# Azure/gpu-provisioner

Measured on AMD Instinct MI355X. Metric: nodeclaims_per_min, higher is better.
Workload: dtype n/a; 1 GPU; model=MI355X NodeClaim provisioning (karpenter CloudProvider contract), vm_sku=Standard_ND128isr_MI355X_v6, concurrent_nodeclaims=8, cloud=in-memory fake AKS, zero latency (BASELINE config #1), apiserver=in-memory, server-side CRD validation on, cycle=create→Launched→Registered→Initialized(amd.com/gpu)→delete→gone, parallelism=single

## Files before the change

### __graft_entry__.py

```python
from __future__ import annotations

import os
import subprocess
import sys
import sysconfig

ROOT = os.path.dirname(os.path.abspath(__file__))
sys.path.insert(0, ROOT)

NATIVE_DIR = os.path.join(ROOT, "gpu_provisioner_amd", "_native")
LIB_PATH = os.path.join(NATIVE_DIR, "libmi355x_nodeagent.so")
HIP_SRC = os.path.join(ROOT, "nodeagent", "agent.hip")
EXTENSIONS = {
    "_jsontree": os.path.join(ROOT, "native", "jsontree.cpp"),
    "_objmodel": os.path.join(ROOT, "native", "objmodel.cpp"),
}


def build() -> None:
    os.makedirs(NATIVE_DIR, exist_ok=True)
    cmd = [
        "hipcc",
        "--offload-arch=gfx950",
        "-O3",
        "-shared",
        "-fPIC",
        HIP_SRC,
        "-o",
        LIB_PATH,
    ]
    print("+", " ".join(cmd), flush=True)
    subprocess.run(cmd, check=True)
    assert os.path.exists(LIB_PATH), f"{LIB_PATH} missing after build"

    for module, src in EXTENSIONS.items():
        ext_path = os.path.join(NATIVE_DIR, module + sysconfig.get_config_var("EXT_SUFFIX"))
        cmd = [
            os.environ.get("CXX", "c++"),
            "-O2",
            "-std=c++17",
            "-shared",
            "-fPIC",
            "-I" + sysconfig.get_paths()["include"],
            src,
            "-o",
            ext_path,
        ]
        print("+", " ".join(cmd), flush=True)
        subprocess.run(cmd, check=True)
        assert os.path.exists(ext_path), f"{ext_path} missing after build"

    import gpu_provisioner_amd
    from gpu_provisioner_amd._native import _jsontree, _objmodel
    from gpu_provisioner_amd.kube import objects

    if os.environ.get("GPU_PROVISIONER_PURE_PYTHON") != "1":
        assert objects.NATIVE_JSONTREE, "native JSON-tree extension built but not in use"
        assert objects.NATIVE_OBJMODEL, "native object-model extension built but not in use"
    from gpu_provisioner_amd.fake.harness import Harness
    from gpu_provisioner_amd.nodeagent import NodeAgent

    print(f"build OK: {LIB_PATH} ({os.path.getsize(LIB_PATH)} bytes)", flush=True)


def smoke() -> None:
    import asyncio

    from gpu_provisioner_amd.apis import v1 as karpv1
    from gpu_provisioner_amd.fake.harness import Harness

    async def provision_cycle() -> None:
        h = Harness(node_wait_interval=0.005).add_all_controllers(
            lifecycle_workers=32, termination_requeue=0.01,
            drain_requeue=0.01, instance_poll=0.01, gc_interval=30.0,
        )
        await h.start()
        try:
            await h.kube.create(h.make_nodeclaim("smoke1"))
            done = await h.wait_initialized("smoke1", timeout=30.0)
            assert karpv1.is_initialized(done), "nodeclaim not initialized"
            assert done["status"]["allocatable"][karpv1.AMD_GPU_RESOURCE] == "8"
            await h.kube.delete(karpv1.API_VERSION, karpv1.KIND_NODECLAIM, "smoke1")
            await h.wait_gone(karpv1.API_VERSION, karpv1.KIND_NODECLAIM, "smoke1", timeout=30.0)
        finally:
            await h.stop()

    asyncio.run(provision_cycle())
    print("smoke: provision+teardown cycle OK", flush=True)

    gpu_available = False
    try:
        import torch

        gpu_available = torch.cuda.is_available()
    except Exception:
        pass
    if gpu_available:
        from gpu_provisioner_amd.nodeagent import NodeAgent

        agent = NodeAgent()
        report = agent.check(bw_bytes=1 << 28)
        assert report.gpu_count >= 1, "no GPUs found by node agent"
        g0 = report.gpus[0]
        assert g0.healthy, f"node agent found problems: {g0.problems}"
        print(
            f"smoke: nodeagent gpu0 {g0.arch} hbm={g0.hbm_gb}GB "
            f"bw={g0.hbm_bw_gbs}GB/s sdma={g0.sdma_bw_gbs}GB/s all-checks=OK",
            flush=True,
        )
    else:
        print("smoke: no GPU present; native nodeagent check skipped", flush=True)


if __name__ == "__main__":
    build()
    smoke()
```

### gpu_provisioner_amd/fake/apiserver.py

```python
from __future__ import annotations

import asyncio
from collections import deque
import itertools
from collections import defaultdict
from typing import Any, AsyncIterator, Callable, Optional

from ..kube import objects as ko
from ..kube.client import (
    ADDED,
    DELETED,
    MODIFIED,
    AlreadyExistsError,
    APIError,
    ConflictError,
    GoneError,
    InvalidError,
    KubeClient,
    LabelSelector,
    NotFoundError,
    json_merge_patch,
    match_field_selector,
    merge_patch_owned,
)

_WATCH_HISTORY = 4096
_WATCH_BROKEN = "__WATCH_BROKEN__"

_SELECTABLE_FIELDS = {
    ("v1", "Pod"): {
        "spec.nodeName",
        "spec.schedulerName",
        "spec.restartPolicy",
        "spec.serviceAccountName",
        "spec.hostNetwork",
        "status.phase",
        "status.podIP",
        "status.nominatedNodeName",
    },
    ("v1", "Node"): {"spec.unschedulable"},
    ("v1", "Namespace"): {"status.phase", "name"},
    ("v1", "Secret"): {"type"},
    ("v1", "Event"): {
        "involvedObject.kind",
        "involvedObject.namespace",
        "involvedObject.name",
        "involvedObject.uid",
        "involvedObject.apiVersion",
        "involvedObject.resourceVersion",
        "involvedObject.fieldPath",
        "reason",
        "reportingComponent",
        "source",
        "type",
    },
}
_GENERIC_FIELDS = {"metadata.name", "metadata.namespace"}


def validate_field_selector(api_version: str, kind: str, selector: str) -> None:
    if not selector:
        return
    allowed = _GENERIC_FIELDS | _SELECTABLE_FIELDS.get((api_version, kind), set())
    for part in selector.split(","):
        part = part.strip()
        if not part:
            continue
        key = part.split("!=" if "!=" in part else "=", 1)[0].strip()
        if key not in allowed:
            raise InvalidError(f"field label not supported: {key}")


def _key(namespace: str, name: str) -> tuple:
    return (namespace or "", name)


def _gvk(api_version: str, kind: str) -> tuple:
    return (api_version, kind)


class InMemoryAPIServer:

    def __init__(self):
        self._store: dict = defaultdict(dict)
        self._rv = itertools.count(1)
        self._lock = asyncio.Lock()
        self._watchers: list = []
        self._history: deque = deque(maxlen=_WATCH_HISTORY)
        self.reactors: list = []
        self.validators: dict = {}
        self.eviction_reactor: Optional[Callable] = None
        self.evictions: list = []


    def _next_rv(self) -> str:
        return str(next(self._rv))

    def _fire_reactors(self, verb: str, gvk: tuple, payload: Any) -> None:
        for r in list(self.reactors):
            err = r(verb, gvk, payload)
            if err is not None:
                raise err

    def _broadcast(self, gvk: tuple, event_type: str, obj: dict) -> None:
        rv = int(obj["metadata"]["resourceVersion"])
        self._history.append((rv, gvk, event_type, obj))
        for wgvk, queue in self._watchers:
            if wgvk == gvk:
                queue.put_nowait((event_type, obj))

    def _bump(self, obj: dict) -> None:
        obj["metadata"]["resourceVersion"] = self._next_rv()

    def _validate(self, gvk: tuple, new: dict, old: Optional[dict]) -> None:
        fn = self.validators.get(gvk)
        if fn is None:
            return
        errs = fn(new, old)
        if errs:
            raise InvalidError(
                f"{gvk[1]} {ko.name_of(new)} is invalid: " + "; ".join(errs[:5])
            )


    async def get(self, api_version: str, kind: str, name: str, namespace: str) -> dict:
        async with self._lock:
            gvk = _gvk(api_version, kind)
            self._fire_reactors("get", gvk, name)
            obj = self._store[gvk].get(_key(namespace, name))
            if obj is None:
                raise NotFoundError(f"{kind} {namespace}/{name} not found")
            return ko.deep_copy(obj)

    async def list(
        self,
        api_version: str,
        kind: str,
        namespace: str,
        label_selector: str,
        field_selector: str,
    ) -> tuple:
        async with self._lock:
            gvk = _gvk(api_version, kind)
            validate_field_selector(api_version, kind, field_selector)
            self._fire_reactors("list", gvk, None)
            sel = LabelSelector.parse(label_selector) if label_selector else None
            out = []
            for (ns, _), obj in self._store[gvk].items():
                if namespace and ns != namespace:
                    continue
                if sel and not sel.matches(ko.labels_of(obj)):
                    continue
                if not match_field_selector(obj, field_selector):
                    continue
                out.append(ko.deep_copy(obj))
            return out, str(self._peek_rv())

    def _peek_rv(self) -> int:
        c = next(self._rv)
        self._rv = itertools.chain([c], self._rv)
        return c - 1

    async def create(self, obj: dict) -> dict:
        async with self._lock:
            api_version, kind = obj.get("apiVersion", ""), obj.get("kind", "")
            if not api_version or not kind or not ko.name_of(obj):
                raise InvalidError("apiVersion, kind and metadata.name are required")
            gvk = _gvk(api_version, kind)
            self._fire_reactors("create", gvk, obj)
            key = _key(ko.namespace_of(obj), ko.name_of(obj))
            if key in self._store[gvk]:
                raise AlreadyExistsError(f"{kind} {key[0]}/{key[1]} already exists")
            stored = ko.deep_copy(obj)
            m = ko.meta(stored)
            m["uid"] = m.get("uid") or ko.uuid4_str()
            m["creationTimestamp"] = m.get("creationTimestamp") or ko.now_rfc3339()
            m["generation"] = 1
            self._validate(gvk, stored, None)
            self._bump(stored)
            self._store[gvk][key] = stored
            if kind == "Event" and len(self._store[gvk]) > 20000:
                drop = next(iter(self._store[gvk]))
                del self._store[gvk][drop]
            self._broadcast(gvk, ADDED, stored)
            return ko.deep_copy(stored)

    async def update(self, obj: dict, subresource: str = "") -> dict:
        async with self._lock:
            api_version, kind = obj.get("apiVersion", ""), obj.get("kind", "")
            gvk = _gvk(api_version, kind)
            self._fire_reactors("update", gvk, obj)
            key = _key(ko.namespace_of(obj), ko.name_of(obj))
            cur = self._store[gvk].get(key)
            if cur is None:
                raise NotFoundError(f"{kind} {key[0]}/{key[1]} not found")
            rv = obj.get("metadata", {}).get("resourceVersion")
            if rv and rv != cur["metadata"]["resourceVersion"]:
                raise ConflictError(
                    f"{kind} {key[1]}: resourceVersion mismatch ({rv} != {cur['metadata']['resourceVersion']})"
                )
            return self._apply_update(gvk, key, cur, obj, subresource)

    def _apply_update(
        self, gvk: tuple, key: tuple, cur: dict, obj: dict, subresource: str, owned: bool = False
    ) -> dict:
        if subresource == "status":
            stored = {**cur, "metadata": {**cur["metadata"]}}
            stored["status"] = ko.deep_copy(obj.get("status", {}))
        else:
            if ko.is_deleting(cur):
                added = set(ko.finalizers_of(obj)) - set(ko.finalizers_of(cur))
                if added:
                    raise InvalidError(
                        "metadata.finalizers: Forbidden: no new finalizers can "
                        f"be added if the object is being deleted (added: {sorted(added)})"
                    )
            new = obj if owned else ko.deep_copy(obj)
            new["status"] = cur.get("status", {})
            nm = ko.meta(new)
            cm = cur["metadata"]
            for f in ("uid", "creationTimestamp", "generation", "deletionTimestamp"):
                if f in cm:
                    nm[f] = cm[f]
                else:
                    nm.pop(f, None)
            ns, cs = new.get("spec"), cur.get("spec")
            if ns is cs:
                pass
            elif ns != cs:
                nm["generation"] = cm.get("generation", 1) + 1
            elif "spec" in new:
                new["spec"] = cs
            stored = new
        self._validate(gvk, stored, cur)
        self._bump(stored)
        if ko.is_deleting(stored) and not ko.finalizers_of(stored) and subresource != "status":
            del self._store[gvk][key]
            self._broadcast(gvk, DELETED, stored)
        else:
            self._store[gvk][key] = stored
            self._broadcast(gvk, MODIFIED, stored)
        return ko.deep_copy(stored)

    async def patch(
        self,
        api_version: str,
        kind: str,
        name: str,
        patch: dict,
        namespace: str,
        subresource: str,
    ) -> dict:
        async with self._lock:
            gvk = _gvk(api_version, kind)
            self._fire_reactors("patch", gvk, name)
            key = _key(namespace, name)
            cur = self._store[gvk].get(key)
            if cur is None:
                raise NotFoundError(f"{kind} {namespace}/{name} not found")
            req_rv = (patch.get("metadata") or {}).get("resourceVersion")
            if req_rv and req_rv != cur["metadata"]["resourceVersion"]:
                raise ConflictError(
                    f"{kind} {name}: resourceVersion mismatch "
                    f"({req_rv} != {cur['metadata']['resourceVersion']})"
                )
            if subresource == "status":
                merged_status = json_merge_patch(cur.get("status", {}), patch.get("status", patch))
                return self._apply_update(gvk, key, cur, {"status": merged_status}, "status")
            merged = merge_patch_owned(cur, patch)
            merged.setdefault("metadata", {})["resourceVersion"] = cur["metadata"]["resourceVersion"]
            return self._apply_update(gvk, key, cur, merged, "", owned=True)

    async def delete(
        self,
        api_version: str,
        kind: str,
        name: str,
        namespace: str,
        uid_precondition: str = "",
        grace_period_seconds: Optional[int] = None,
    ) -> None:
        async with self._lock:
            gvk = _gvk(api_version, kind)
            self._fire_reactors("delete", gvk, name)
            key = _key(namespace, name)
            cur = self._store[gvk].get(key)
            if cur is None:
                raise NotFoundError(f"{kind} {namespace}/{name} not found")
            if uid_precondition and ko.uid_of(cur) != uid_precondition:
                raise ConflictError(f"{kind} {name}: uid precondition failed")
            if ko.finalizers_of(cur):
                if not ko.is_deleting(cur):
                    stored = {**cur, "metadata": {**cur["metadata"]}}
                    ko.meta(stored)["deletionTimestamp"] = ko.now_rfc3339()
                    self._bump(stored)
                    self._store[gvk][key] = stored
                    self._broadcast(gvk, MODIFIED, stored)
                return
            stored = {**cur, "metadata": {**cur["metadata"]}}
            ko.meta(stored)["deletionTimestamp"] = ko.now_rfc3339()
            self._bump(stored)
            del self._store[gvk][key]
            self._broadcast(gvk, DELETED, stored)

    async def evict(self, pod: dict, grace_period_seconds: Optional[int]) -> None:
        async with self._lock:
            if self.eviction_reactor is not None:
                err = self.eviction_reactor(pod)
                if err is not None:
                    raise err
            gvk = _gvk("v1", "Pod")
            key = _key(ko.namespace_of(pod), ko.name_of(pod))
            cur = self._store[gvk].get(key)
            if cur is None:
                raise NotFoundError(f"Pod {key[0]}/{key[1]} not found")
            self.evictions.append(key)
            stored = ko.deep_copy(cur)
            ko.meta(stored)["deletionTimestamp"] = ko.now_rfc3339()
            self._bump(stored)
            if ko.finalizers_of(cur):
                self._store[gvk][key] = stored
                self._broadcast(gvk, MODIFIED, stored)
            else:
                del self._store[gvk][key]
                self._broadcast(gvk, DELETED, stored)

    def subscribe(self, api_version: str, kind: str, resource_version: str) -> tuple:
        gvk = _gvk(api_version, kind)
        queue: asyncio.Queue = asyncio.Queue()
        if resource_version:
            rv = int(resource_version)
            if self._history:
                oldest = self._history[0][0]
                if rv + 1 < oldest and any(True for _ in self._store[gvk]):
                    raise GoneError(f"resourceVersion {rv} too old")
            for erv, egvk, etype, eobj in self._history:
                if egvk == gvk and erv > rv:
                    queue.put_nowait((etype, ko.deep_copy(eobj)))
        entry = (gvk, queue)
        self._watchers.append(entry)

        def unsubscribe():
            try:
                self._watchers.remove(entry)
            except ValueError:
                pass

        return queue, unsubscribe

    def break_watches(self) -> int:
        broken = 0
        for _, queue in list(self._watchers):
            queue.put_nowait((_WATCH_BROKEN, None))
            broken += 1
        return broken


class InMemoryClient(KubeClient):

    def __init__(self, server: InMemoryAPIServer):
        self.server = server

    async def get(self, api_version: str, kind: str, name: str, namespace: str = "") -> dict:
        return await self.server.get(api_version, kind, name, namespace)

    async def list(
        self,
# ... 78 lines not shown
```

### native/jsontree.cpp

```cpp
#define PY_SSIZE_T_CLEAN
#include <Python.h>

namespace {


inline bool is_container(PyObject* o) {
    return PyDict_CheckExact(o) || PyList_CheckExact(o);
}

PyObject* copy_tree(PyObject* o) {
    if (PyDict_CheckExact(o)) {
        if (Py_EnterRecursiveCall(" while copying a JSON tree")) return nullptr;
        PyObject* out = PyDict_Copy(o);
        if (out != nullptr) {
            Py_ssize_t pos = 0;
            PyObject *k, *v;
            while (PyDict_Next(out, &pos, &k, &v)) {
                if (!is_container(v)) continue;
                PyObject* nv = copy_tree(v);
                if (nv == nullptr || PyDict_SetItem(out, k, nv) < 0) {
                    Py_XDECREF(nv);
                    Py_CLEAR(out);
                    break;
                }
                Py_DECREF(nv);
            }
        }
        Py_LeaveRecursiveCall();
        return out;
    }
    if (PyList_CheckExact(o)) {
        if (Py_EnterRecursiveCall(" while copying a JSON tree")) return nullptr;
        PyObject* out = PyList_GetSlice(o, 0, PyList_GET_SIZE(o));
        if (out != nullptr) {
            Py_ssize_t n = PyList_GET_SIZE(out);
            for (Py_ssize_t i = 0; i < n; i++) {
                PyObject* v = PyList_GET_ITEM(out, i);
                if (!is_container(v)) continue;
                PyObject* nv = copy_tree(v);
                if (nv == nullptr) {
                    Py_CLEAR(out);
                    break;
                }
                PyList_SET_ITEM(out, i, nv);
                Py_DECREF(v);
            }
        }
        Py_LeaveRecursiveCall();
        return out;
    }
    Py_INCREF(o);
    return o;
}

PyObject* py_deep_copy(PyObject*, PyObject* obj) { return copy_tree(obj); }


PyObject* dict_of(PyObject* target) {
    if (target == nullptr || !PyDict_Check(target)) return PyDict_New();
    if (PyDict_CheckExact(target)) return PyDict_Copy(target);
    return PyObject_CallOneArg((PyObject*)&PyDict_Type, target);
}

PyObject* merge(PyObject* target, PyObject* patch, bool owned);

int merge_item(PyObject* out, PyObject* k, PyObject* v, bool owned) {
    if (v == Py_None) {
        if (PyDict_DelItem(out, k) < 0) {
            if (!PyErr_ExceptionMatches(PyExc_KeyError)) return -1;
            PyErr_Clear();
        }
        return 0;
    }
    PyObject* nv;
    if (PyDict_Check(v)) {
        PyObject* sub = PyDict_GetItemWithError(out, k);
        if (sub == nullptr && PyErr_Occurred()) return -1;
        Py_XINCREF(sub);
        nv = merge(sub, v, owned);
        Py_XDECREF(sub);
    } else if (owned) {
        nv = copy_tree(v);
    } else {
        Py_INCREF(v);
        nv = v;
    }
    if (nv == nullptr) return -1;
    int rc = PyDict_SetItem(out, k, nv);
    Py_DECREF(nv);
    return rc;
}

PyObject* merge(PyObject* target, PyObject* patch, bool owned) {
    if (!PyDict_Check(patch)) {
        if (owned) return copy_tree(patch);
        Py_INCREF(patch);
        return patch;
    }
    if (Py_EnterRecursiveCall(" while applying a merge patch")) return nullptr;
    PyObject* out = dict_of(target);
    if (out != nullptr) {
        bool ok = true;
        if (PyDict_CheckExact(patch)) {
            Py_ssize_t pos = 0;
            PyObject *k, *v;
            while (ok && PyDict_Next(patch, &pos, &k, &v)) {
                Py_INCREF(k);
                Py_INCREF(v);
                ok = merge_item(out, k, v, owned) == 0;
                Py_DECREF(k);
                Py_DECREF(v);
            }
        } else {
            PyObject* items = PyObject_CallMethod(patch, "items", nullptr);
            PyObject* it = items ? PyObject_GetIter(items) : nullptr;
            Py_XDECREF(items);
            ok = it != nullptr;
            PyObject* kv;
            while (ok && (kv = PyIter_Next(it)) != nullptr) {
                PyObject* seq = PySequence_Fast(kv, "items() must yield pairs");
                Py_DECREF(kv);
                if (seq == nullptr || PySequence_Fast_GET_SIZE(seq) != 2) {
                    if (seq != nullptr) PyErr_SetString(PyExc_ValueError, "items() must yield pairs");
                    Py_XDECREF(seq);
                    ok = false;
                    break;
                }
                ok = merge_item(out, PySequence_Fast_GET_ITEM(seq, 0),
                                PySequence_Fast_GET_ITEM(seq, 1), owned) == 0;
                Py_DECREF(seq);
            }
            if (ok && PyErr_Occurred()) ok = false;
            Py_XDECREF(it);
        }
        if (!ok) Py_CLEAR(out);
    }
    Py_LeaveRecursiveCall();
    return out;
}

PyObject* py_json_merge_patch(PyObject*, PyObject* const* args, Py_ssize_t nargs) {
    if (nargs != 2) {
        PyErr_SetString(PyExc_TypeError, "json_merge_patch(target, patch) takes 2 arguments");
        return nullptr;
    }
    return merge(args[0], args[1], false);
}

PyObject* str_metadata;

PyObject* py_merge_patch_owned(PyObject*, PyObject* const* args, Py_ssize_t nargs) {
    if (nargs != 2) {
        PyErr_SetString(PyExc_TypeError, "merge_patch_owned(cur, patch) takes 2 arguments");
        return nullptr;
    }
    PyObject* cur = args[0];
    PyObject* out = merge(cur, args[1], true);
    if (out == nullptr || !PyDict_CheckExact(out) || !PyDict_Check(cur)) return out;
    PyObject* m = PyDict_GetItemWithError(out, str_metadata);
    if (m == nullptr) {
        if (PyErr_Occurred()) Py_CLEAR(out);
        return out;
    }
    if (PyDict_CheckExact(m) && m == PyDict_GetItemWithError(cur, str_metadata)) {
        PyObject* fresh = PyDict_Copy(m);
        if (fresh == nullptr || PyDict_SetItem(out, str_metadata, fresh) < 0) Py_CLEAR(out);
        Py_XDECREF(fresh);
    } else if (PyErr_Occurred()) {
        Py_CLEAR(out);
    }
    return out;
}


struct Names {
    PyObject *type, *properties, *additionalProperties, *preserve, *required, *items,
        *maxItems, *enum_set, *enum_, *pattern_re, *pattern, *maxLength, *minLength,
        *minimum, *maximum, *anyOf, *search, *spec, *status, *nodeClassRef, *group,
        *kind, *name, *empty;
} S;

inline PyObject* sget(PyObject* schema, PyObject* key) {
    PyObject* v = PyDict_GetItemWithError(schema, key);
    if (v == nullptr) PyErr_Clear();
    return v;
}

inline PyObject* sget2(PyObject* schema, PyObject* overlay, PyObject* key) {
    if (overlay != nullptr) {
        PyObject* v = sget(overlay, key);
        if (v != nullptr) return v;
    }
    return sget(schema, key);
}

inline bool is_str(PyObject* o, const char* s) {
    return o != nullptr && PyUnicode_CheckExact(o) && PyUnicode_CompareWithASCIIString(o, s) == 0;
}

int len_cmp(Py_ssize_t n, PyObject* limit, int op) {
    PyObject* pn = PyLong_FromSsize_t(n);
    if (pn == nullptr) return -1;
    int r = PyObject_RichCompareBool(pn, limit, op);
    Py_DECREF(pn);
    return r;
}

int validate(PyObject* obj, PyObject* schema, PyObject* overlay);

int validate_changed(PyObject* nw, PyObject* old, PyObject* schema);

int check_required(PyObject* obj, PyObject* schema) {
    PyObject* req = sget(schema, S.required);
    if (req == nullptr) return 1;
    if (!PyList_CheckExact(req) && !PyTuple_CheckExact(req)) return 0;
    Py_ssize_t n = PySequence_Fast_GET_SIZE(req);
    for (Py_ssize_t i = 0; i < n; i++) {
        int has = PyDict_Contains(obj, PySequence_Fast_GET_ITEM(req, i));
        if (has <= 0) return has;
    }
    return 1;
}

int validate_string(PyObject* obj, PyObject* schema, PyObject* overlay) {
    if (!PyUnicode_Check(obj)) return 0;
    if (!PyUnicode_CheckExact(obj)) return 0;
    PyObject* enum_set = sget2(schema, overlay, S.enum_set);
    if (enum_set != nullptr && enum_set != Py_None) {
        int in = PySequence_Contains(enum_set, obj);
        if (in <= 0) return in;
    } else {
        PyObject* en = sget2(schema, overlay, S.enum_);
        if (en != nullptr) {
            int in = PySequence_Contains(en, obj);
            if (in <= 0) return in;
        }
    }
    PyObject* pat = sget2(schema, overlay, S.pattern_re);
    if (pat != nullptr && pat != Py_None) {
        PyObject* m = PyObject_CallMethodOneArg(pat, S.search, obj);
        if (m == nullptr) return -1;
        bool miss = m == Py_None;
        Py_DECREF(m);
        if (miss) return 0;
    } else if (sget2(schema, overlay, S.pattern) != nullptr) {
        return 0;
    }
    PyObject* lim = sget2(schema, overlay, S.maxLength);
    if (lim != nullptr) {
        int r = len_cmp(PyUnicode_GET_LENGTH(obj), lim, Py_GT);
        if (r != 0) return r < 0 ? -1 : 0;
    }
    lim = sget2(schema, overlay, S.minLength);
    if (lim != nullptr) {
// ... 317 lines not shown
```

Before: 103,100 NodeClaims/min.

## Move in-memory apiserver verb success paths into a native C++ revision store

Adds a native _revstore extension that runs the common success paths of get, create, update, patch and delete directly on the store dicts, covering key lookup, precondition checks, merge, validation, resourceVersion bump, history and watcher broadcast. Any case it cannot handle returns NotImplemented and falls back to the Python body. The resourceVersion counter becomes a plain int, and the reactor loop is skipped when no reactors are registered. The merge and copy helpers are moved into a shared header. The aim is to cut Python interpreter overhead per API call, at the cost of a large duplicated native code path that could drift from the Python semantics.

```diff
diff --git a/__graft_entry__.py b/__graft_entry__.py
--- a/__graft_entry__.py
+++ b/__graft_entry__.py
@@ -14,6 +14,7 @@
 EXTENSIONS = {
     "_jsontree": os.path.join(ROOT, "native", "jsontree.cpp"),
     "_objmodel": os.path.join(ROOT, "native", "objmodel.cpp"),
+    "_revstore": os.path.join(ROOT, "native", "revstore.cpp"),
 }
 
 
@@ -51,12 +52,14 @@
         assert os.path.exists(ext_path), f"{ext_path} missing after build"
 
     import gpu_provisioner_amd
-    from gpu_provisioner_amd._native import _jsontree, _objmodel
+    from gpu_provisioner_amd._native import _jsontree, _objmodel, _revstore
+    from gpu_provisioner_amd.fake import apiserver
     from gpu_provisioner_amd.kube import objects
 
     if os.environ.get("GPU_PROVISIONER_PURE_PYTHON") != "1":
         assert objects.NATIVE_JSONTREE, "native JSON-tree extension built but not in use"
         assert objects.NATIVE_OBJMODEL, "native object-model extension built but not in use"
+        assert apiserver.NATIVE_REVSTORE, "native revision-store extension built but not in use"
     from gpu_provisioner_amd.fake.harness import Harness
     from gpu_provisioner_amd.nodeagent import NodeAgent
 
diff --git a/gpu_provisioner_amd/fake/apiserver.py b/gpu_provisioner_amd/fake/apiserver.py
--- a/gpu_provisioner_amd/fake/apiserver.py
+++ b/gpu_provisioner_amd/fake/apiserver.py
@@ -1,8 +1,8 @@
 from __future__ import annotations
 
 import asyncio
+import os
 from collections import deque
-import itertools
 from collections import defaultdict
 from typing import Any, AsyncIterator, Callable, Optional
 
@@ -26,6 +26,17 @@
 
 _WATCH_HISTORY = 4096
 _WATCH_BROKEN = "__WATCH_BROKEN__"
+_EVENT_CAP = 20000
+
+_native_revstore = None
+if os.environ.get("GPU_PROVISIONER_PURE_PYTHON") != "1":
+    try:
+        from .._native import _revstore as _native_revstore
+    except ImportError:
+        _native_revstore = None
+NATIVE_REVSTORE = _native_revstore is not None
+if NATIVE_REVSTORE:
+    _native_revstore.set_helpers(ko.uuid4_str, ko.now_rfc3339)
 
 _SELECTABLE_FIELDS = {
     ("v1", "Pod"): {
@@ -83,7 +94,9 @@
 
     def __init__(self):
         self._store: dict = defaultdict(dict)
-        self._rv = itertools.count(1)
+        self._rv = 0
+        self._native = _native_revstore
+        self._event_cap = _EVENT_CAP
         self._lock = asyncio.Lock()
         self._watchers: list = []
         self._history: deque = deque(maxlen=_WATCH_HISTORY)
@@ -94,7 +107,8 @@
 
 
     def _next_rv(self) -> str:
-        return str(next(self._rv))
+        self._rv += 1
+        return str(self._rv)
 
     def _fire_reactors(self, verb: str, gvk: tuple, payload: Any) -> None:
         for r in list(self.reactors):
@@ -103,8 +117,7 @@
                 raise err
 
     def _broadcast(self, gvk: tuple, event_type: str, obj: dict) -> None:
-        rv = int(obj["metadata"]["resourceVersion"])
-        self._history.append((rv, gvk, event_type, obj))
+        self._history.append((self._rv, gvk, event_type, obj))
         for wgvk, queue in self._watchers:
             if wgvk == gvk:
                 queue.put_nowait((event_type, obj))
@@ -125,8 +138,13 @@
 
     async def get(self, api_version: str, kind: str, name: str, namespace: str) -> dict:
         async with self._lock:
-            gvk = _gvk(api_version, kind)
-            self._fire_reactors("get", gvk, name)
+            gvk = (api_version, kind)
+            if self.reactors:
+                self._fire_reactors("get", gvk, name)
+            if self._native is not None:
+                out = self._native.get(self._store[gvk], namespace, name)
+                if out is not NotImplemented:
+                    return out
             obj = self._store[gvk].get(_key(namespace, name))
             if obj is None:
                 raise NotFoundError(f"{kind} {namespace}/{name} not found")
@@ -157,17 +175,22 @@
             return out, str(self._peek_rv())
 
     def _peek_rv(self) -> int:
-        c = next(self._rv)
-        self._rv = itertools.chain([c], self._rv)
-        return c - 1
+        return self._rv
 
     async def create(self, obj: dict) -> dict:
         async with self._lock:
             api_version, kind = obj.get("apiVersion", ""), obj.get("kind", "")
             if not api_version or not kind or not ko.name_of(obj):
                 raise InvalidError("apiVersion, kind and metadata.name are required")
-            gvk = _gvk(api_version, kind)
-            self._fire_reactors("create", gvk, obj)
+            gvk = (api_version, kind)
+            if self.reactors:
+                self._fire_reactors("create", gvk, obj)
+            if self._native is not None:
+                out = self._native.create(
+                    self, gvk, self._store[gvk], obj, self.validators.get(gvk), self._event_cap
+                )
+                if out is not NotImplemented:
+                    return out
             key = _key(ko.namespace_of(obj), ko.name_of(obj))
             if key in self._store[gvk]:
                 raise AlreadyExistsError(f"{kind} {key[0]}/{key[1]} already exists")
@@ -179,7 +202,7 @@
             self._validate(gvk, stored, None)
             self._bump(stored)
             self._store[gvk][key] = stored
-            if kind == "Event" and len(self._store[gvk]) > 20000:
+            if kind == "Event" and len(self._store[gvk]) > self._event_cap:
                 drop = next(iter(self._store[gvk]))
                 del self._store[gvk][drop]
             self._broadcast(gvk, ADDED, stored)
@@ -188,8 +211,15 @@
     async def update(self, obj: dict, subresource: str = "") -> dict:
         async with self._lock:
             api_version, kind = obj.get("apiVersion", ""), obj.get("kind", "")
-            gvk = _gvk(api_version, kind)
-            self._fire_reactors("update", gvk, obj)
+            gvk = (api_version, kind)
+            if self.reactors:
+                self._fire_reactors("update", gvk, obj)
+            if self._native is not None:
+                out = self._native.update(
+                    self, gvk, self._store[gvk], obj, subresource, self.validators.get(gvk)
+                )
+                if out is not NotImplemented:
+                    return out
             key = _key(ko.namespace_of(obj), ko.name_of(obj))
             cur = self._store[gvk].get(key)
             if cur is None:
@@ -252,8 +282,16 @@
         subresource: str,
     ) -> dict:
         async with self._lock:
-            gvk = _gvk(api_version, kind)
-            self._fire_reactors("patch", gvk, name)
+            gvk = (api_version, kind)
+            if self.reactors:
+                self._fire_reactors("patch", gvk, name)
+            if self._native is not None:
+                out = self._native.patch(
+                    self, gvk, self._store[gvk], namespace, name, patch, subresource,
+                    self.validators.get(gvk),
+                )
+                if out is not NotImplemented:
+                    return out
             key = _key(namespace, name)
             cur = self._store[gvk].get(key)
             if cur is None:
@@ -281,8 +319,15 @@
         grace_period_seconds: Optional[int] = None,
     ) -> None:
         async with self._lock:
-            gvk = _gvk(api_version, kind)
-            self._fire_reactors("delete", gvk, name)
+            gvk = (api_version, kind)
+            if self.reactors:
+                self._fire_reactors("delete", gvk, name)
+            if self._native is not None:
+                out = self._native.delete(
+                    self, gvk, self._store[gvk], namespace, name, uid_precondition
+                )
+                if out is not NotImplemented:
+                    return out
             key = _key(namespace, name)
             cur = self._store[gvk].get(key)
             if cur is None:
diff --git a/native/jsontree.cpp b/native/jsontree.cpp
--- a/native/jsontree.cpp
+++ b/native/jsontree.cpp
@@ -1,143 +1,15 @@
 #define PY_SSIZE_T_CLEAN
 #include <Python.h>
 
+#include "jsontree_walk.h"
+
 namespace {
 
-
-inline bool is_container(PyObject* o) {
-    return PyDict_CheckExact(o) || PyList_CheckExact(o);
-}
-
-PyObject* copy_tree(PyObject* o) {
-    if (PyDict_CheckExact(o)) {
-        if (Py_EnterRecursiveCall(" while copying a JSON tree")) return nullptr;
-        PyObject* out = PyDict_Copy(o);
-        if (out != nullptr) {
-            Py_ssize_t pos = 0;
-            PyObject *k, *v;
-            while (PyDict_Next(out, &pos, &k, &v)) {
-                if (!is_container(v)) continue;
-                PyObject* nv = copy_tree(v);
-                if (nv == nullptr || PyDict_SetItem(out, k, nv) < 0) {
-                    Py_XDECREF(nv);
-                    Py_CLEAR(out);
-                    break;
-                }
-                Py_DECREF(nv);
-            }
-        }
-        Py_LeaveRecursiveCall();
-        return out;
-    }
-    if (PyList_CheckExact(o)) {
-        if (Py_EnterRecursiveCall(" while copying a JSON tree")) return nullptr;
-        PyObject* out = PyList_GetSlice(o, 0, PyList_GET_SIZE(o));
-        if (out != nullptr) {
-            Py_ssize_t n = PyList_GET_SIZE(out);
-            for (Py_ssize_t i = 0; i < n; i++) {
-                PyObject* v = PyList_GET_ITEM(out, i);
-                if (!is_container(v)) continue;
-                PyObject* nv = copy_tree(v);
-                if (nv == nullptr) {
-                    Py_CLEAR(out);
-                    break;
-                }
-                PyList_SET_ITEM(out, i, nv);
-                Py_DECREF(v);
-            }
-        }
-        Py_LeaveRecursiveCall();
-        return out;
-    }
-    Py_INCREF(o);
-    return o;
-}
+using jsontree_walk::copy_tree;
+using jsontree_walk::merge;
+using jsontree_walk::merge_owned;
 
 PyObject* py_deep_copy(PyObject*, PyObject* obj) { return copy_tree(obj); }
-
-
-PyObject* dict_of(PyObject* target) {
-    if (target == nullptr || !PyDict_Check(target)) return PyDict_New();
-    if (PyDict_CheckExact(target)) return PyDict_Copy(target);
-    return PyObject_CallOneArg((PyObject*)&PyDict_Type, target);
-}
-
-PyObject* merge(PyObject* target, PyObject* patch, bool owned);
-
-int merge_item(PyObject* out, PyObject* k, PyObject* v, bool owned) {
-    if (v == Py_None) {
-        if (PyDict_DelItem(out, k) < 0) {
-            if (!PyErr_ExceptionMatches(PyExc_KeyError)) return -1;
-            PyErr_Clear();
-        }
-        return 0;
-    }
-    PyObject* nv;
-    if (PyDict_Check(v)) {
-        PyObject* sub = PyDict_GetItemWithError(out, k);
-        if (sub == nullptr && PyErr_Occurred()) return -1;
-        Py_XINCREF(sub);
-        nv = merge(sub, v, owned);
-        Py_XDECREF(sub);
-    } else if (owned) {
-        nv = copy_tree(v);
-    } else {
-        Py_INCREF(v);
-        nv = v;
-    }
-    if (nv == nullptr) return -1;
-    int rc = PyDict_SetItem(out, k, nv);
-    Py_DECREF(nv);
-    return rc;
-}
-
-PyObject* merge(PyObject* target, PyObject* patch, bool owned) {
-    if (!PyDict_Check(patch)) {
-        if (owned) return copy_tree(patch);
-        Py_INCREF(patch);
-        return patch;
-    }
-    if (Py_EnterRecursiveCall(" while applying a merge patch")) return nullptr;
-    PyObject* out = dict_of(target);
-    if (out != nullptr) {
-        bool ok = true;
-        if (PyDict_CheckExact(patch)) {
-            Py_ssize_t pos = 0;
-            PyObject *k, *v;
-            while (ok && PyDict_Next(patch, &pos, &k, &v)) {
-                Py_INCREF(k);
-                Py_INCREF(v);
-                ok = merge_item(out, k, v, owned) == 0;
-                Py_DECREF(k);
-                Py_DECREF(v);
-            }
-        } else {
-            PyObject* items = PyObject_CallMethod(patch, "items", nullptr);
-            PyObject* it = items ? PyObject_GetIter(items) : nullptr;
-            Py_XDECREF(items);
-            ok = it != nullptr;
-            PyObject* kv;
-            while (ok && (kv = PyIter_Next(it)) != nullptr) {
-                PyObject* seq = PySequence_Fast(kv, "items() must yield pairs");
-                Py_DECREF(kv);
-                if (seq == nullptr || PySequence_Fast_GET_SIZE(seq) != 2) {
-                    if (seq != nullptr) PyErr_SetString(PyExc_ValueError, "items() must yield pairs");
-                    Py_XDECREF(seq);
-                    ok = false;
-                    break;
-                }
-                ok = merge_item(out, PySequence_Fast_GET_ITEM(seq, 0),
-                                PySequence_Fast_GET_ITEM(seq, 1), owned) == 0;
-                Py_DECREF(seq);
-            }
-            if (ok && PyErr_Occurred()) ok = false;
-            Py_XDECREF(it);
-        }
-        if (!ok) Py_CLEAR(out);
-    }
-    Py_LeaveRecursiveCall();
-    return out;
-}
 
 PyObject* py_json_merge_patch(PyObject*, PyObject* const* args, Py_ssize_t nargs) {
     if (nargs != 2) {
@@ -154,22 +26,7 @@
         PyErr_SetString(PyExc_TypeError, "merge_patch_owned(cur, patch) takes 2 arguments");
         return nullptr;
     }
-    PyObject* cur = args[0];
-    PyObject* out = merge(cur, args[1], true);
-    if (out == nullptr || !PyDict_CheckExact(out) || !PyDict_Check(cur)) return out;
-    PyObject* m = PyDict_GetItemWithError(out, str_metadata);
-    if (m == nullptr) {
-        if (PyErr_Occurred()) Py_CLEAR(out);
-        return out;
-    }
-    if (PyDict_CheckExact(m) && m == PyDict_GetItemWithError(cur, str_metadata)) {
-        PyObject* fresh = PyDict_Copy(m);
-        if (fresh == nullptr || PyDict_SetItem(out, str_metadata, fresh) < 0) Py_CLEAR(out);
-        Py_XDECREF(fresh);
-    } else if (PyErr_Occurred()) {
-        Py_CLEAR(out);
-    }
-    return out;
+    return merge_owned(args[0], args[1], str_metadata);
 }
 
 
diff --git a/native/jsontree_walk.h b/native/jsontree_walk.h
--- /dev/null
+++ b/native/jsontree_walk.h
@@ -0,0 +1,163 @@
+#ifndef GPU_PROVISIONER_AMD_JSONTREE_WALK_H
+#define GPU_PROVISIONER_AMD_JSONTREE_WALK_H
+
+#define PY_SSIZE_T_CLEAN
+#include <Python.h>
+
+namespace jsontree_walk {
+
+
+static inline bool is_container(PyObject* o) {
+    return PyDict_CheckExact(o) || PyList_CheckExact(o);
+}
+
+static inline PyObject* copy_tree(PyObject* o) {
+    if (PyDict_CheckExact(o)) {
+        if (Py_EnterRecursiveCall(" while copying a JSON tree")) return nullptr;
+        PyObject* out = PyDict_Copy(o);
+        if (out != nullptr) {
+            Py_ssize_t pos = 0;
+            PyObject *k, *v;
+            while (PyDict_Next(out, &pos, &k, &v)) {
+                if (!is_container(v)) continue;
+                PyObject* nv = copy_tree(v);
+                if (nv == nullptr || PyDict_SetItem(out, k, nv) < 0) {
+                    Py_XDECREF(nv);
+                    Py_CLEAR(out);
+                    break;
+                }
+                Py_DECREF(nv);
+            }
+        }
+        Py_LeaveRecursiveCall();
+        return out;
+    }
+    if (PyList_CheckExact(o)) {
+        if (Py_EnterRecursiveCall(" while copying a JSON tree")) return nullptr;
+        PyObject* out = PyList_GetSlice(o, 0, PyList_GET_SIZE(o));
+        if (out != nullptr) {
+            Py_ssize_t n = PyList_GET_SIZE(out);
+            for (Py_ssize_t i = 0; i < n; i++) {
+                PyObject* v = PyList_GET_ITEM(out, i);
+                if (!is_container(v)) continue;
+                PyObject* nv = copy_tree(v);
+                if (nv == nullptr) {
+                    Py_CLEAR(out);
+                    break;
+                }
+                PyList_SET_ITEM(out, i, nv);
+                Py_DECREF(v);
+            }
+        }
+        Py_LeaveRecursiveCall();
+        return out;
+    }
+    Py_INCREF(o);
+    return o;
+}
+
+
+static inline PyObject* dict_of(PyObject* target) {
+    if (target == nullptr || !PyDict_Check(target)) return PyDict_New();
+    if (PyDict_CheckExact(target)) return PyDict_Copy(target);
+    return PyObject_CallOneArg((PyObject*)&PyDict_Type, target);
+}
+
+static inline PyObject* merge(PyObject* target, PyObject* patch, bool owned);
+
+static inline int merge_item(PyObject* out, PyObject* k, PyObject* v, bool owned) {
+    if (v == Py_None) {
+        if (PyDict_DelItem(out, k) < 0) {
+            if (!PyErr_ExceptionMatches(PyExc_KeyError)) return -1;
+            PyErr_Clear();
+        }
+        return 0;
+    }
+    PyObject* nv;
+    if (PyDict_Check(v)) {
+        PyObject* sub = PyDict_GetItemWithError(out, k);
+        if (sub == nullptr && PyErr_Occurred()) return -1;
+        Py_XINCREF(sub);
+        nv = merge(sub, v, owned);
+        Py_XDECREF(sub);
+    } else if (owned) {
+        nv = copy_tree(v);
+    } else {
+        Py_INCREF(v);
+        nv = v;
+    }
+    if (nv == nullptr) return -1;
+    int rc = PyDict_SetItem(out, k, nv);
+    Py_DECREF(nv);
+    return rc;
+}
+
+static inline PyObject* merge(PyObject* target, PyObject* patch, bool owned) {
+    if (!PyDict_Check(patch)) {
+        if (owned) return copy_tree(patch);
+        Py_INCREF(patch);
+        return patch;
+    }
+    if (Py_EnterRecursiveCall(" while applying a merge patch")) return nullptr;
+    PyObject* out = dict_of(target);
+    if (out != nullptr) {
+        bool ok = true;
+        if (PyDict_CheckExact(patch)) {
+            Py_ssize_t pos = 0;
+            PyObject *k, *v;
+            while (ok && PyDict_Next(patch, &pos, &k, &v)) {
+                Py_INCREF(k);
+                Py_INCREF(v);
+                ok = merge_item(out, k, v, owned) == 0;
+                Py_DECREF(k);
+                Py_DECREF(v);
+            }
+        } else {
+            PyObject* items = PyObject_CallMethod(patch, "items", nullptr);
+            PyObject* it = items ? PyObject_GetIter(items) : nullptr;
+            Py_XDECREF(items);
+            ok = it != nullptr;
+            PyObject* kv;
+            while (ok && (kv = PyIter_Next(it)) != nullptr) {
+                PyObject* seq = PySequence_Fast(kv, "items() must yield pairs");
+                Py_DECREF(kv);
+                if (seq == nullptr || PySequence_Fast_GET_SIZE(seq) != 2) {
+                    if (seq != nullptr) PyErr_SetString(PyExc_ValueError, "items() must yield pairs");
+                    Py_XDECREF(seq);
+                    ok = false;
+                    break;
+                }
+                ok = merge_item(out, PySequence_Fast_GET_ITEM(seq, 0),
+                                PySequence_Fast_GET_ITEM(seq, 1), owned) == 0;
+                Py_DECREF(seq);
+            }
+            if (ok && PyErr_Occurred()) ok = false;
+            Py_XDECREF(it);
+        }
+        if (!ok) Py_CLEAR(out);
+    }
+    Py_LeaveRecursiveCall();
+    return out;
+}
+
+static inline PyObject* merge_owned(PyObject* cur, PyObject* patch, PyObject* str_metadata) {
+    PyObject* out = merge(cur, patch, true);
+    if (out == nullptr || !PyDict_CheckExact(out) || !PyDict_Check(cur)) return out;
+    PyObject* m = PyDict_GetItemWithError(out, str_metadata);
+    if (m == nullptr) {
+        if (PyErr_Occurred()) Py_CLEAR(out);
+        return out;
+    }
+    if (PyDict_CheckExact(m) && m == PyDict_GetItemWithError(cur, str_metadata)) {
+        PyObject* fresh = PyDict_Copy(m);
+        if (fresh == nullptr || PyDict_SetItem(out, str_metadata, fresh) < 0) Py_CLEAR(out);
+        Py_XDECREF(fresh);
+    } else if (PyErr_Occurred()) {
+        Py_CLEAR(out);
+    }
+    return out;
+}
+
+}
+
+#endif
diff --git a/native/revstore.cpp b/native/revstore.cpp
--- /dev/null
+++ b/native/revstore.cpp
@@ -0,0 +1,544 @@
+#define PY_SSIZE_T_CLEAN
+#include <Python.h>
+
+#include <limits.h>
+
+#include "jsontree_walk.h"
+
+namespace {
+
+using jsontree_walk::copy_tree;
+using jsontree_walk::merge;
+using jsontree_walk::merge_owned;
+
+struct Names {
+    PyObject *metadata, *name, *namespace_, *uid, *creationTimestamp, *generation,
+        *deletionTimestamp, *finalizers, *resourceVersion, *spec, *status, *empty, *Event,
+        *ADDED, *MODIFIED, *DELETED, *rv_attr, *history_attr, *watchers_attr, *append,
+        *put_nowait;
+} S;
+
+PyObject* long_one;
+PyObject* uuid4_str;
+PyObject* now_rfc3339;
+
+struct Ref {
+    PyObject* p;
+    explicit Ref(PyObject* o = nullptr) : p(o) {}
+    ~Ref() { Py_XDECREF(p); }
+    Ref(const Ref&) = delete;
+    Ref& operator=(const Ref&) = delete;
+    void reset(PyObject* o) { Py_XSETREF(p, o); }
+    PyObject* release() {
+        PyObject* o = p;
+        p = nullptr;
+        return o;
+    }
+    operator PyObject*() const { return p; }
+};
+
+inline PyObject* newref(PyObject* o) {
+    Py_XINCREF(o);
+    return o;
+}
+
+inline PyObject* miss() { Py_RETURN_NOTIMPLEMENTED; }
+
+inline int look(PyObject* d, PyObject* key, PyObject** out) {
+    *out = PyDict_GetItemWithError(d, key);
+    if (*out != nullptr) return 1;
+    return PyErr_Occurred() ? -1 : 0;
+}
+
+inline int truthy(PyObject* d, PyObject* key) {
+    PyObject* v;
+    int r = look(d, key, &v);
+    if (r <= 0) return r;
+    Ref hold(newref(v));
+    return PyObject_IsTrue(v);
+}
+
+inline bool str_eq(PyObject* a, PyObject* b) {
+    return a == b || PyUnicode_Compare(a, b) == 0;
+}
+
+PyObject* make_key(PyObject* ns, PyObject* name) {
+    if (ns == nullptr || ns == Py_None) ns = S.empty;
+    if (name == nullptr || !PyUnicode_CheckExact(ns) || !PyUnicode_CheckExact(name)) return nullptr;
+    return PyTuple_Pack(2, ns, name);
+}
+
+int current(PyObject* bucket, PyObject* key, PyObject** cur, PyObject** cm) {
+    int r = look(bucket, key, cur);
+    if (r <= 0) return r;
+    if (!PyDict_CheckExact(*cur)) return 0;
+    r = look(*cur, S.metadata, cm);
+    if (r == 1 && !PyDict_CheckExact(*cm)) return 0;
+    return r;
+}
+
+int rv_precondition(PyObject* meta, PyObject* cm) {
+    PyObject* want = nullptr;
+    if (meta != nullptr && look(meta, S.resourceVersion, &want) < 0) return -1;
+    if (want == nullptr || want == Py_None) return 1;
+    if (!PyUnicode_CheckExact(want)) return 0;
+    if (PyUnicode_GET_LENGTH(want) == 0) return 1;
+    PyObject* have;
+    int r = look(cm, S.resourceVersion, &have);
+    if (r <= 0) return r;
+    return PyUnicode_CheckExact(have) && str_eq(want, have);
+}
+
+int no_new_finalizers(PyObject* nm, PyObject* cm) {
+    PyObject *nf, *cf;
+    if (look(nm, S.finalizers, &nf) < 0 || look(cm, S.finalizers, &cf) < 0) return -1;
+    if (nf == nullptr || nf == Py_None) return 1;
+    if (cf == Py_None) cf = nullptr;
+    if (!PyList_CheckExact(nf) || (cf != nullptr && !PyList_CheckExact(cf))) return 0;
+    for (Py_ssize_t i = 0; i < PyList_GET_SIZE(nf); i++) {
+        PyObject* f = PyList_GET_ITEM(nf, i);
+        if (!PyUnicode_CheckExact(f)) return 0;
+        bool found = false;
+        for (Py_ssize_t j = 0; !found && cf != nullptr && j < PyList_GET_SIZE(cf); j++) {
+            PyObject* c = PyList_GET_ITEM(cf, j);
+            if (!PyUnicode_CheckExact(c)) return 0;
+            found = str_eq(f, c);
+        }
+        if (!found) return 0;
+    }
+    return 1;
+}
+
+int valid(PyObject* validator, PyObject* nw, PyObject* old) {
+    if (validator == Py_None) return 1;
+    PyObject* args[2] = {nw, old};
+    Ref errs(PyObject_Vectorcall(validator, args, 2, nullptr));
+    if (errs == nullptr) return -1;
+    int t = PyObject_IsTrue(errs);
+    return t < 0 ? -1 : !t;
+}
+
+
+struct Sink {
+    Ref append;
+    Ref watchers;
+    long long rv = 0;
+};
+
+int open_sink(PyObject* server, Sink& s) {
+    Ref rv(PyObject_GetAttr(server, S.rv_attr));
+    Ref hist(rv != nullptr ? PyObject_GetAttr(server, S.history_attr) : nullptr);
+    if (hist != nullptr) s.append.reset(PyObject_GetAttr(hist, S.append));
+    if (s.append != nullptr) s.watchers.reset(PyObject_GetAttr(server, S.watchers_attr));
+    if (s.watchers == nullptr) {
+        PyErr_Clear();
+        return 0;
+    }
+    PyObject* ws = s.watchers.p;
+    if (!PyLong_CheckExact(rv.p) || !PyList_CheckExact(ws)) return 0;
+    int overflow = 0;
+    s.rv = PyLong_AsLongLongAndOverflow(rv.p, &overflow);
+    if (overflow || s.rv < 0 || s.rv == LLONG_MAX) return 0;
+    for (Py_ssize_t i = 0; i < PyList_GET_SIZE(ws); i++) {
+        PyObject* w = PyList_GET_ITEM(ws, i);
+        if (!PyTuple_CheckExact(w) || PyTuple_GET_SIZE(w) != 2) return 0;
+    }
+    return 1;
+}
+
+int commit(PyObject* server, Sink& s, PyObject* gvk, PyObject* bucket, PyObject* key,
+           PyObject* stored, PyObject* nm, PyObject* event_type, bool remove,
+           Py_ssize_t cap = -1) {
+    long long n = s.rv + 1;
+    Ref rv_str(PyUnicode_FromFormat("%lld", n));
+    Ref rv_int(PyLong_FromLongLong(n));
+    if (rv_str == nullptr || rv_int == nullptr) return -1;
+    Ref entry(PyTuple_Pack(4, (PyObject*)rv_int, gvk, event_type, stored));
+    Ref event(PyTuple_Pack(2, event_type, stored));
+    if (entry == nullptr || event == nullptr) return -1;
+    if (PyDict_SetItem(nm, S.resourceVersion, rv_str) < 0) return -1;
+    if (PyObject_SetAttr(server, S.rv_attr, rv_int) < 0) return -1;
+    if ((remove ? PyDict_DelItem(bucket, key) : PyDict_SetItem(bucket, key, stored)) < 0) return -1;
+    if (cap >= 0 && PyDict_GET_SIZE(bucket) > cap) {
+        Py_ssize_t pos = 0;
+        PyObject *k, *v;
+        if (PyDict_Next(bucket, &pos, &k, &v)) {
+            Ref oldest(newref(k));
+            if (PyDict_DelItem(bucket, oldest) < 0) return -1;
+        }
+    }
+    Ref appended(PyObject_CallOneArg(s.append, entry));
+    if (appended == nullptr) return -1;
+    PyObject* ws = s.watchers.p;
+    for (Py_ssize_t i = 0; i < PyList_GET_SIZE(ws); i++) {
+        PyObject* w = PyList_GET_ITEM(ws, i);
+        if (!PyTuple_CheckExact(w) || PyTuple_GET_SIZE(w) != 2) continue;
+        Ref hold(newref(w));
+        int eq = PyObject_RichCompareBool(PyTuple_GET_ITEM(w, 0), gvk, Py_EQ);
+        if (eq < 0) return -1;
+        if (!eq) continue;
+        Ref put(PyObject_CallMethodOneArg(PyTuple_GET_ITEM(w, 1), S.put_nowait, event));
+        if (put == nullptr) return -1;
+    }
+    return 0;
+}
+
+
+enum Mode {
+    STATUS,
+    STATUS_OWNED,
+    MAIN,
+    MAIN_OWNED,
+};
+
+PyObject* apply_update(PyObject* server, PyObject* gvk, PyObject* bucket, PyObject* key,
+                       PyObject* cur, PyObject* cm, PyObject* obj, Mode mode,
+                       PyObject* validator) {
+    Sink sink;
+    if (!open_sink(server, sink)) return miss();
+    Ref stored, meta_ref;
+    bool remove = false;
+    if (mode == STATUS || mode == STATUS_OWNED) {
+        stored.reset(PyDict_Copy(cur));
+        meta_ref.reset(PyDict_Copy(cm));
+        if (stored == nullptr || meta_ref == nullptr) return nullptr;
+        Ref status;
+        if (mode == STATUS_OWNED) {
+            status.reset(newref(obj));
+        } else {
+            PyObject* v;
+            if (look(obj, S.status, &v) < 0) return nullptr;
+            status.reset(v != nullptr ? copy_tree(v) : PyDict_New());
+        }
+        if (status == nullptr || PyDict_SetItem(stored, S.metadata, meta_ref) < 0 ||
+            PyDict_SetItem(stored, S.status, status) < 0)
+            return nullptr;
+    } else {
+        PyObject* om;
+        int r = look(obj, S.metadata, &om);
+        if (r < 0) return nullptr;
+        if (r == 0 || !PyDict_CheckExact(om)) return miss();
+        int deleting = truthy(cm, S.deletionTimestamp);
+        if (deleting < 0) return nullptr;
+        if (deleting) {
+            r = no_new_finalizers(om, cm);
+            if (r < 0) return nullptr;
+            if (r == 0) return miss();
+        }
+        stored.reset(mode == MAIN_OWNED ? newref(obj) : copy_tree(obj));
+        if (stored == nullptr) return nullptr;
+        PyObject* v;
+        if (look(cur, S.status, &v) < 0) return nullptr;
+        Ref status(v != nullptr ? newref(v) : PyDict_New());
+        if (status == nullptr || PyDict_SetItem(stored, S.status, status) < 0) return nullptr;
+        if (look(stored, S.metadata, &v) <= 0) return nullptr;
+        meta_ref.reset(newref(v));
+        PyObject* fixed[4] = {S.uid, S.creationTimestamp, S.generation, S.deletionTimestamp};
+        for (PyObject* f : fixed) {
+            if (look(cm, f, &v) < 0) return nullptr;
+            if (v != nullptr) {
+                if (PyDict_SetItem(meta_ref, f, v) < 0) return nullptr;
+            } else {
+                int has = PyDict_Contains(meta_ref, f);
+                if (has < 0 || (has && PyDict_DelItem(meta_ref, f) < 0)) return nullptr;
+            }
+        }
+        PyObject *ns, *cs;
+        if (look(stored, S.spec, &ns) < 0 || look(cur, S.spec, &cs) < 0) return nullptr;
+        PyObject* a = ns != nullptr ? ns : Py_None;
+        PyObject* b = cs != nullptr ? cs : Py_None;
+        if (a != b) {
+            int ne = PyObject_RichCompareBool(a, b, Py_NE);
+            if (ne < 0) return nullptr;
+            if (ne) {
+                PyObject* gen;
+                if (look(cm, S.generation, &gen) < 0) return nullptr;
+                if (gen == nullptr) gen = long_one;
+                if (!PyLong_CheckExact(gen)) return miss();
+                Ref next(PyNumber_Add(gen, long_one));
+                if (next == nullptr || PyDict_SetItem(meta_ref, S.generation, next) < 0) return nullptr;
+            } else if (ns != nullptr && cs != nullptr) {
+                if (PyDict_SetItem(stored, S.spec, cs) < 0) return nullptr;
+            }
+        }
+    }
+    int ok = valid(validator, stored, cur);
+    if (ok < 0) return nullptr;
+    if (!ok) return miss();
+    if (mode == MAIN || mode == MAIN_OWNED) {
+        int deleting = truthy(meta_ref, S.deletionTimestamp);
+        int fins = deleting > 0 ? truthy(meta_ref, S.finalizers) : 0;
+        if (deleting < 0 || fins < 0) return nullptr;
+        remove = deleting && !fins;
+    }
+    if (commit(server, sink, gvk, bucket, key, stored, meta_ref, remove ? S.DELETED : S.MODIFIED,
+               remove) < 0)
+        return nullptr;
+    return copy_tree(stored);
+}
+
+inline bool is_gvk(PyObject* gvk) { return PyTuple_CheckExact(gvk) && PyTuple_GET_SIZE(gvk) == 2; }
+
+inline int subresource_mode(PyObject* sub) {
+    if (!PyUnicode_CheckExact(sub)) return -1;
+    if (PyUnicode_GET_LENGTH(sub) == 0) return MAIN;
+    return str_eq(sub, S.status) ? STATUS : -1;
+}
+
+
+PyObject* py_get(PyObject*, PyObject* const* args, Py_ssize_t nargs) {
+    if (nargs != 3) {
+        PyErr_SetString(PyExc_TypeError, "get(bucket, namespace, name) takes 3 arguments");
+        return nullptr;
+    }
+    if (!PyDict_Check(args[0])) return miss();
+    Ref key(make_key(args[1], args[2]));
+    if (key == nullptr) return PyErr_Occurred() ? nullptr : miss();
+    PyObject* obj;
+    int r = look(args[0], key, &obj);
+    if (r < 0) return nullptr;
+    if (r == 0) return miss();
+    return copy_tree(obj);
+}
+
+PyObject* py_create(PyObject*, PyObject* const* args, Py_ssize_t nargs) {
+    if (nargs != 6) {
+        PyErr_SetString(PyExc_TypeError,
+                        "create(server, gvk, bucket, obj, validator, event_cap) takes 6 arguments");
+        return nullptr;
+    }
+    PyObject *server = args[0], *gvk = args[1], *bucket = args[2], *obj = args[3],
+             *validator = args[4];
+    Py_ssize_t cap = PyLong_AsSsize_t(args[5]);
+    if (cap == -1 && PyErr_Occurred()) return nullptr;
+    if (!is_gvk(gvk) || !PyDict_Check(bucket) || !PyDict_CheckExact(obj) || uuid4_str == nullptr)
+        return miss();
+    PyObject* om;
+    int r = look(obj, S.metadata, &om);
+    if (r < 0) return nullptr;
+    if (r == 0 || !PyDict_CheckExact(om)) return miss();
+    PyObject *name, *ns;
+    if (look(om, S.name, &name) < 0 || look(om, S.namespace_, &ns) < 0) return nullptr;
+    if (name == nullptr || !PyUnicode_CheckExact(name) || PyUnicode_GET_LENGTH(name) == 0)
+        return miss();
+    Ref key(make_key(ns, name));
+    if (key == nullptr) return PyErr_Occurred() ? nullptr : miss();
+    r = PyDict_Contains(bucket, key);
+    if (r < 0) return nullptr;
+    if (r) return miss();
+    Sink sink;
+    if (!open_sink(server, sink)) return miss();
+
+    Ref stored(copy_tree(obj));
+    if (stored == nullptr) return nullptr;
+    PyObject* m;
+    if (look(stored, S.metadata, &m) <= 0) return nullptr;
+    Ref meta_ref(newref(m));
+    struct { PyObject* key; PyObject* make; } fill[2] = {
+        {S.uid, uuid4_str}, {S.creationTimestamp, now_rfc3339}};
+    for (auto& f : fill) {
+        int has = truthy(meta_ref, f.key);
+        if (has < 0) return nullptr;
+        if (has) continue;
+        Ref v(PyObject_CallNoArgs(f.make));
+        if (v == nullptr || PyDict_SetItem(meta_ref, f.key, v) < 0) return nullptr;
+    }
+    if (PyDict_SetItem(meta_ref, S.generation, long_one) < 0) return nullptr;
+    int ok = valid(validator, stored, Py_None);
+    if (ok < 0) return nullptr;
+    if (!ok) return miss();
+    PyObject* kind = PyTuple_GET_ITEM(gvk, 1);
+    bool capped = PyUnicode_CheckExact(kind) && str_eq(kind, S.Event);
+    if (commit(server, sink, gvk, bucket, key, stored, meta_ref, S.ADDED, false,
+               capped ? cap : -1) < 0)
+        return nullptr;
+    return copy_tree(stored);
+}
+
+PyObject* py_update(PyObject*, PyObject* const* args, Py_ssize_t nargs) {
+    if (nargs != 6) {
+        PyErr_SetString(PyExc_TypeError,
+                        "update(server, gvk, bucket, obj, subresource, validator) takes 6 arguments");
+        return nullptr;
+    }
+    PyObject *server = args[0], *gvk = args[1], *bucket = args[2], *obj = args[3];
+    int mode = subresource_mode(args[4]);
+    if (mode < 0 || !is_gvk(gvk) || !PyDict_Check(bucket) || !PyDict_CheckExact(obj)) return miss();
+    PyObject* om;
+    int r = look(obj, S.metadata, &om);
+    if (r < 0) return nullptr;
+    if (r == 0 || !PyDict_CheckExact(om)) return miss();
+    PyObject *name, *ns;
+    if (look(om, S.name, &name) < 0 || look(om, S.namespace_, &ns) < 0) return nullptr;
+    Ref key(make_key(ns, name));
+    if (key == nullptr) return PyErr_Occurred() ? nullptr : miss();
+    PyObject *cur, *cm;
+    r = current(bucket, key, &cur, &cm);
+    if (r < 0) return nullptr;
+    if (r == 0) return miss();
+    Ref hold_cur(newref(cur)), hold_cm(newref(cm));
+    r = rv_precondition(om, cm);
+    if (r < 0) return nullptr;
+    if (r == 0) return miss();
+    return apply_update(server, gvk, bucket, key, cur, cm, obj, (Mode)mode, args[5]);
+}
+
+PyObject* py_patch(PyObject*, PyObject* const* args, Py_ssize_t nargs) {
+    if (nargs != 8) {
+        PyErr_SetString(PyExc_TypeError,
+                        "patch(server, gvk, bucket, namespace, name, patch, subresource, validator) "
+                        "takes 8 arguments");
+        return nullptr;
+    }
+    PyObject *server = args[0], *gvk = args[1], *bucket = args[2], *patch = args[5];
+    int mode = subresource_mode(args[6]);
+    if (mode < 0 || !is_gvk(gvk) || !PyDict_Check(bucket) || !PyDict_CheckExact(patch)) return miss();
+    Ref key(make_key(args[3], args[4]));
+    if (key == nullptr) return PyErr_Occurred() ? nullptr : miss();
+    PyObject *cur, *cm;
+    int r = current(bucket, key, &cur, &cm);
+    if (r < 0) return nullptr;
+    if (r == 0) return miss();
+    Ref hold_cur(newref(cur)), hold_cm(newref(cm));
+    PyObject* pm;
+    r = look(patch, S.metadata, &pm);
+    if (r < 0) return nullptr;
+    if (r == 1 && !PyDict_CheckExact(pm)) return miss();
+    r = rv_precondition(pm, cm);
+    if (r < 0) return nullptr;
+    if (r == 0) return miss();
+    if (mode == STATUS) {
+        PyObject *sp, *cs;
+        if (look(patch, S.status, &sp) < 0 || look(cur, S.status, &cs) < 0) return nullptr;
+        Ref merged(merge(cs, sp != nullptr ? sp : patch, true));
+        if (merged == nullptr) return nullptr;
+        return apply_update(server, gvk, bucket, key, cur, cm, merged, STATUS_OWNED, args[7]);
+    }
+    PyObject* rv;
+    r = look(cm, S.resourceVersion, &rv);
+    if (r < 0) return nullptr;
+    if (r == 0) return miss();
+    Ref merged(merge_owned(cur, patch, S.metadata));
+    if (merged == nullptr) return nullptr;
+    PyObject* mm;
+    r = PyDict_CheckExact(merged.p) ? look(merged, S.metadata, &mm) : 0;
+    if (r < 0) return nullptr;
+    if (r == 0 || !PyDict_CheckExact(mm)) return miss();
+    if (PyDict_SetItem(mm, S.resourceVersion, rv) < 0) return nullptr;
+    return apply_update(server, gvk, bucket, key, cur, cm, merged, MAIN_OWNED, args[7]);
+}
+
+PyObject* py_delete(PyObject*, PyObject* const* args, Py_ssize_t nargs) {
+    if (nargs != 6) {
+        PyErr_SetString(PyExc_TypeError,
+                        "delete(server, gvk, bucket, namespace, name, uid_precondition) takes 6 arguments");
+        return nullptr;
+    }
+    PyObject *server = args[0], *gvk = args[1], *bucket = args[2], *want_uid = args[5];
+    if (!is_gvk(gvk) || !PyDict_Check(bucket) || !PyUnicode_CheckExact(want_uid) ||
+        now_rfc3339 == nullptr)
+        return miss();
+    Ref key(make_key(args[3], args[4]));
+    if (key == nullptr) return PyErr_Occurred() ? nullptr : miss();
+    PyObject *cur, *cm;
+    int r = current(bucket, key, &cur, &cm);
+    if (r < 0) return nullptr;
+    if (r == 0) return miss();
+    Ref hold_cur(newref(cur)), hold_cm(newref(cm));
+    if (PyUnicode_GET_LENGTH(want_uid) > 0) {
+        PyObject* uid;
+        if (look(cm, S.uid, &uid) < 0) return nullptr;
+        if (uid == nullptr) uid = S.empty;
+        if (!PyUnicode_CheckExact(uid) || !str_eq(uid, want_uid)) return miss();
+    }
+    int fins = truthy(cm, S.finalizers);
+    int deleting = fins > 0 ? truthy(cm, S.deletionTimestamp) : 0;
+    if (fins < 0 || deleting < 0) return nullptr;
+    if (fins && deleting) Py_RETURN_NONE;
+    Sink sink;
+    if (!open_sink(server, sink)) return miss();
+    Ref stored(PyDict_Copy(cur)), nm(PyDict_Copy(cm));
+    Ref now(PyObject_CallNoArgs(now_rfc3339));
+    if (stored == nullptr || nm == nullptr || now == nullptr ||
+        PyDict_SetItem(stored, S.metadata, nm) < 0 ||
+        PyDict_SetItem(nm, S.deletionTimestamp, now) < 0)
+        return nullptr;
+    if (commit(server, sink, gvk, bucket, key, stored, nm, fins ? S.MODIFIED : S.DELETED, !fins) < 0)
+        return nullptr;
+    Py_RETURN_NONE;
+}
+
+PyObject* py_set_helpers(PyObject*, PyObject* const* args, Py_ssize_t nargs) {
+    if (nargs != 2 || !PyCallable_Check(args[0]) || !PyCallable_Check(args[1])) {
+        PyErr_SetString(PyExc_TypeError, "set_helpers(uuid4_str, now_rfc3339) takes two callables");
+        return nullptr;
+    }
+    Py_XSETREF(uuid4_str, newref(args[0]));
+    Py_XSETREF(now_rfc3339, newref(args[1]));
+    Py_RETURN_NONE;
+}
+
+#define FAST(f) (PyCFunction)(void (*)(void))f, METH_FASTCALL
+
+PyMethodDef methods[] = {
+    {"set_helpers", FAST(py_set_helpers),
+     "set_helpers(uuid4_str, now_rfc3339): bind the uid and clock functions create and delete call."},
+    {"get", FAST(py_get), "get(bucket, namespace, name): a copy of the stored revision."},
+    {"create", FAST(py_create),
+     "create(server, gvk, bucket, obj, validator, event_cap): store a new object, return a copy."},
+    {"update", FAST(py_update),
+     "update(server, gvk, bucket, obj, subresource, validator): replace the main resource or the "
+     "status, return a copy."},
+    {"patch", FAST(py_patch),
+     "patch(server, gvk, bucket, namespace, name, patch, subresource, validator): merge patch the "
+     "main resource or the status, return a copy."},
+    {"delete", FAST(py_delete),
+     "delete(server, gvk, bucket, namespace, name, uid_precondition): mark deleting or remove."},
+    {nullptr, nullptr, 0, nullptr},
+};
+
+PyModuleDef moduledef = {
+    PyModuleDef_HEAD_INIT, "_revstore",
+    "Native success path of the in-memory apiserver's verbs; every entry point returns "
+    "NotImplemented, with nothing touched, for what the Python body has to handle.",
+    -1, methods, nullptr, nullptr, nullptr, nullptr,
+};
+
+bool intern_names() {
+    struct { PyObject** slot; const char* text; } table[] = {
+        {&S.metadata, "metadata"},
+        {&S.name, "name"},
+        {&S.namespace_, "namespace"},
+        {&S.uid, "uid"},
+        {&S.creationTimestamp, "creationTimestamp"},
+        {&S.generation, "generation"},
+        {&S.deletionTimestamp, "deletionTimestamp"},
+        {&S.finalizers, "finalizers"},
+        {&S.resourceVersion, "resourceVersion"},
+        {&S.spec, "spec"},
+        {&S.status, "status"},
+        {&S.empty, ""},
+        {&S.Event, "Event"},
+        {&S.ADDED, "ADDED"},
+        {&S.MODIFIED, "MODIFIED"},
+        {&S.DELETED, "DELETED"},
+        {&S.rv_attr, "_rv"},
+        {&S.history_attr, "_history"},
+        {&S.watchers_attr, "_watchers"},
+        {&S.append, "append"},
+        {&S.put_nowait, "put_nowait"},
+    };
+    for (auto& e : table) {
+        *e.slot = PyUnicode_InternFromString(e.text);
+        if (*e.slot == nullptr) return false;
+    }
+    long_one = PyLong_FromLong(1);
+    return long_one != nullptr;
+}
+
+}
+
+PyMODINIT_FUNC PyInit__revstore(void) {
+    if (!intern_names()) return nullptr;
+    return PyModule_Create(&moduledef);
+}
```

Measured after the change: 115,100 NodeClaims/min, median of 6. +11.7%, better.
